# borodark/exmc

Hardware: AMD Instinct MI355X
Metric: leapfrog_steps_per_s (higher is better)
Workload: dtype f64; 1 GPU; eight_schools d=10, 4096 chains/GPU (4096 total), 138450 draws/chain (2769 steps of 50 draws) after one shared 1000-iteration warmup, max_tree_depth 10, target_accept 0.8; draws_per_chain=138450, lanes_per_chain=16, warmup_lanes_per_chain=16, seed=42

## Files before the change

### exmc_amd/csrc/exmc_device.hpp

```cpp
#pragma once

#include <hip/hip_runtime.h>
#include <stdint.h>
#include <type_traits>

#include <utility>

#include "../../include/exmc_detmath.h"

namespace exmc {

constexpr uint64_t kMask58 = (1ULL << 58) - 1;

#ifndef EXMC_FIXED_PART_PIECES
#define EXMC_FIXED_PART_PIECES 7
#endif

__device__ __forceinline__ bool div_in_range(double x) {
  const uint32_t h = (uint32_t)__double2hiint(x) & 0x7fffffffu;
  return (h - 0x28300000u) < (0x57C00000u - 0x28300000u);
}

struct Recip {
  double b, r;
};

__device__ __forceinline__ Recip make_recip(double b) { return Recip{b, exmc_rcp_refined(b)}; }

__device__ __forceinline__ Recip make_recip_literal(double b) {
  __asm__ volatile("" : "+v"(b));
  return make_recip(b);
}

template <bool kFast>
struct Div {
  bool ok = true;
  __device__ __forceinline__ void watch(double x) {
    if (kFast) ok = ok && div_in_range(x);
  }
  __device__ __forceinline__ void watch_if(bool relevant, double x) {
    if (kFast) ok = ok && (!relevant || div_in_range(x));
  }
  template <int ELO, int EHI>
  __device__ __forceinline__ void watch_exp_if(bool relevant, double x) {
    static_assert(ELO >= -380 && EHI <= 380 && ELO < EHI, "inside the division window");
    if (kFast) {
      const uint32_t h = (uint32_t)__double2hiint(x) & 0x7fffffffu;
      const bool in = (h - ((uint32_t)(1023 + ELO) << 20)) < ((uint32_t)(EHI - ELO) << 20);
      ok = ok && (!relevant || in);
    }
  }
  __device__ __forceinline__ double operator()(double a, const Recip& c) const {
    return kFast ? exmc_div_core(a, c.b, c.r) : (a / c.b);
  }
  __device__ __forceinline__ double operator()(double a, double b) const {
    return kFast ? exmc_div_core(a, b, exmc_rcp_refined(b)) : (a / b);
  }
};

template <class F>
__device__ __forceinline__ double with_fast_div(F&& f) {
  Div<true> fast;
  double r = f(fast);
  if (__builtin_expect(__any(fast.ok ? 0 : 1) != 0, 0)) {
    Div<false> exact;
    r = f(exact);
  }
  return r;
}

constexpr int kDppXor1 = 0xB1;
constexpr int kDppXor2 = 0x4E;
constexpr int kDppHalfMirror = 0x141;
constexpr int kDppRowMirror = 0x140;

template <int CTRL>
__device__ __forceinline__ double dpp_move(double v) {
  int lo = __double2loint(v), hi = __double2hiint(v);
  lo = __builtin_amdgcn_mov_dpp(lo, CTRL, 0xF, 0xF, true);
  hi = __builtin_amdgcn_mov_dpp(hi, CTRL, 0xF, 0xF, true);
  return __hiloint2double(hi, lo);
}

__device__ __forceinline__ double readlane_f64(double v, int lane) {
  int lo = __builtin_amdgcn_readlane(__double2loint(v), lane);
  int hi = __builtin_amdgcn_readlane(__double2hiint(v), lane);
  return __hiloint2double(hi, lo);
}

template <int G, int N>
__device__ __forceinline__ void xgroup_sum_n(double (&s)[N]) {
  static_assert(G == 16 || G == 32, "two or four lane groups per wavefront");
#pragma unroll
  for (int k = 0; k < N; k++) {
    double t = readlane_f64(s[k], 0);
#pragma unroll
    for (int j = 1; j < 64 / G; j++) t = t + readlane_f64(s[k], j * G);
    s[k] = t;
  }
}

#ifndef EXMC_XROW_PERMLANE
#define EXMC_XROW_PERMLANE 1
#endif
__device__ __forceinline__ double sum_xor16(double v) {
#if EXMC_XROW_PERMLANE
  const unsigned lo = (unsigned)__double2loint(v), hi = (unsigned)__double2hiint(v);
  const auto rl = __builtin_amdgcn_permlane16_swap(lo, lo, false, false);
  const auto rh = __builtin_amdgcn_permlane16_swap(hi, hi, false, false);
  return __hiloint2double((int)rh[0], (int)rl[0]) + __hiloint2double((int)rh[1], (int)rl[1]);
#else
  const int a = (((int)threadIdx.x & 63) ^ 16) << 2;
  return v + __hiloint2double(__builtin_amdgcn_ds_bpermute(a, __double2hiint(v)),
                              __builtin_amdgcn_ds_bpermute(a, __double2loint(v)));
#endif
}
__device__ __forceinline__ double sum_xor32(double v) {
#if EXMC_XROW_PERMLANE
  const unsigned lo = (unsigned)__double2loint(v), hi = (unsigned)__double2hiint(v);
  const auto rl = __builtin_amdgcn_permlane32_swap(lo, lo, false, false);
  const auto rh = __builtin_amdgcn_permlane32_swap(hi, hi, false, false);
  return __hiloint2double((int)rh[0], (int)rl[0]) + __hiloint2double((int)rh[1], (int)rl[1]);
#else
  const int a = (((int)threadIdx.x & 63) ^ 32) << 2;
  return v + __hiloint2double(__builtin_amdgcn_ds_bpermute(a, __double2hiint(v)),
                              __builtin_amdgcn_ds_bpermute(a, __double2loint(v)));
#endif
}
__device__ __forceinline__ double swap_xor16(double v) {
#if EXMC_XROW_PERMLANE
  const unsigned lo = (unsigned)__double2loint(v), hi = (unsigned)__double2hiint(v);
  const auto rl = __builtin_amdgcn_permlane16_swap(lo, lo, false, false);
  const auto rh = __builtin_amdgcn_permlane16_swap(hi, hi, false, false);
  return (threadIdx.x & 16) ? __hiloint2double((int)rh[0], (int)rl[0]) : __hiloint2double((int)rh[1], (int)rl[1]);
#else
  const int a = (((int)threadIdx.x & 63) ^ 16) << 2;
  return __hiloint2double(__builtin_amdgcn_ds_bpermute(a, __double2hiint(v)),
                          __builtin_amdgcn_ds_bpermute(a, __double2loint(v)));
#endif
}
__device__ __forceinline__ double swap_xor32(double v) {
#if EXMC_XROW_PERMLANE
  const unsigned lo = (unsigned)__double2loint(v), hi = (unsigned)__double2hiint(v);
  const auto rl = __builtin_amdgcn_permlane32_swap(lo, lo, false, false);
  const auto rh = __builtin_amdgcn_permlane32_swap(hi, hi, false, false);
  return (threadIdx.x & 32) ? __hiloint2double((int)rh[0], (int)rl[0]) : __hiloint2double((int)rh[1], (int)rl[1]);
#else
  const int a = (((int)threadIdx.x & 63) ^ 32) << 2;
  return __hiloint2double(__builtin_amdgcn_ds_bpermute(a, __double2hiint(v)),
                          __builtin_amdgcn_ds_bpermute(a, __double2loint(v)));
#endif
}

template <int N>
__device__ __forceinline__ void wave_scan_fwd(double (&v)[N]) {
  const int lane = threadIdx.x & 63, lr = lane & 15;
#define EXMC_SCAN_STAGE(DD)                                                       \
  _Pragma("unroll") for (int k = 0; k < N; k++) {                               \
    const double m = dpp_move<0x110 + DD>(v[k]);                  \
    v[k] = (lr >= DD) ? v[k] + m : v[k];                                          \
// ... 105 lines not shown
#endif
}

template <int G, bool kLds = false>
__device__ __forceinline__ double group_allsum(double v) {
  double a[1] = {v};
  group_allsum_n<G, 1, kLds>(a);
  return a[0];
}

template <int G, int D>
inline constexpr bool kSeqSum = (G == 16 && D <= 12);

#define EXMC_FMAC_B(A, V, I) \
  "v_fmac_f64_dpp %[" #A "], %[" #V "], %[one] row_newbcast:" #I " row_mask:0xf bank_mask:0xf\n\t"
#define EXMC_SEQ1(I) EXMC_FMAC_B(a0, v0, I)
#define EXMC_SEQ2(I) EXMC_SEQ1(I) EXMC_FMAC_B(a1, v1, I)
#define EXMC_SEQ3(I) EXMC_SEQ2(I) EXMC_FMAC_B(a2, v2, I)
#define EXMC_SEQ6(I) EXMC_SEQ3(I) EXMC_FMAC_B(a3, v3, I) EXMC_FMAC_B(a4, v4, I) EXMC_FMAC_B(a5, v5, I)
#define EXMC_LANES_1(S) S(0)
#define EXMC_LANES_2(S) EXMC_LANES_1(S) S(1)
#define EXMC_LANES_3(S) EXMC_LANES_2(S) S(2)
#define EXMC_LANES_4(S) EXMC_LANES_3(S) S(3)
#define EXMC_LANES_5(S) EXMC_LANES_4(S) S(4)
#define EXMC_LANES_6(S) EXMC_LANES_5(S) S(5)
#define EXMC_LANES_7(S) EXMC_LANES_6(S) S(6)
#define EXMC_LANES_8(S) EXMC_LANES_7(S) S(7)
#define EXMC_LANES_9(S) EXMC_LANES_8(S) S(8)
#define EXMC_LANES_10(S) EXMC_LANES_9(S) S(9)
#define EXMC_LANES_11(S) EXMC_LANES_10(S) S(10)
#define EXMC_LANES_12(S) EXMC_LANES_11(S) S(11)
#define EXMC_SEQSUM_ASM_H(HEAD, SEQ, OUTS, INS)                                              \
  if constexpr (NL == 1) __asm__(HEAD EXMC_LANES_1(SEQ) : OUTS : INS);                         \
  else if constexpr (NL == 2) __asm__(HEAD EXMC_LANES_2(SEQ) : OUTS : INS);                    \
  else if constexpr (NL == 3) __asm__(HEAD EXMC_LANES_3(SEQ) : OUTS : INS);                    \
  else if constexpr (NL == 4) __asm__(HEAD EXMC_LANES_4(SEQ) : OUTS : INS);                    \
  else if constexpr (NL == 5) __asm__(HEAD EXMC_LANES_5(SEQ) : OUTS : INS);                    \
  else if constexpr (NL == 6) __asm__(HEAD EXMC_LANES_6(SEQ) : OUTS : INS);                    \
  else if constexpr (NL == 7) __asm__(HEAD EXMC_LANES_7(SEQ) : OUTS : INS);                    \
  else if constexpr (NL == 8) __asm__(HEAD EXMC_LANES_8(SEQ) : OUTS : INS);                    \
  else if constexpr (NL == 9) __asm__(HEAD EXMC_LANES_9(SEQ) : OUTS : INS);                    \
  else if constexpr (NL == 10) __asm__(HEAD EXMC_LANES_10(SEQ) : OUTS : INS);                  \
  else if constexpr (NL == 11) __asm__(HEAD EXMC_LANES_11(SEQ) : OUTS : INS);                  \
  else __asm__(HEAD EXMC_LANES_12(SEQ) : OUTS : INS);
#define EXMC_NOP2 "s_nop 1\n\t"
#define EXMC_COMMA ,

__device__ __forceinline__ double seq_one() { return 1.0; }

template <int NL>
__device__ __forceinline__ void row_seqsum(double& a0, double v0) {
  static_assert(NL >= 1 && NL <= 12, "lanes of one DPP row, where the chain beats the butterfly");
  const double one = seq_one();
  EXMC_SEQSUM_ASM_H(EXMC_NOP2, EXMC_SEQ1, [a0] "+v"(a0), [v0] "v"(v0) EXMC_COMMA [one] "v"(one))
}
template <int NL>
__device__ __forceinline__ void row_seqsum(double& a0, double& a1, double v0, double v1) {
  const double one = seq_one();
  EXMC_SEQSUM_ASM_H(EXMC_NOP2, EXMC_SEQ2, [a0] "+v"(a0) EXMC_COMMA [a1] "+v"(a1),
                  [v0] "v"(v0) EXMC_COMMA [v1] "v"(v1) EXMC_COMMA [one] "v"(one))
}
template <int NL>
__device__ __forceinline__ void row_seqsum(double& a0, double& a1, double& a2, double v0, double v1,
                                           double v2) {
  const double one = seq_one();
  EXMC_SEQSUM_ASM_H(EXMC_NOP2, EXMC_SEQ3, [a0] "+v"(a0) EXMC_COMMA [a1] "+v"(a1) EXMC_COMMA [a2] "+v"(a2),
                  [v0] "v"(v0) EXMC_COMMA [v1] "v"(v1) EXMC_COMMA [v2] "v"(v2) EXMC_COMMA [one] "v"(one))
}
#define EXMC_FMAC_R(A, V, I) \
  "v_fmac_f64_dpp %[" #A "], %[" #V "], %[one] row_newbcast:%[l" #I "] row_mask:0xf bank_mask:0xf\n\t"
#define EXMC_SEQ3R(I) EXMC_FMAC_R(a0, v0, I) EXMC_FMAC_R(a1, v1, I) EXMC_FMAC_R(a2, v2, I)
#define EXMC_LANE_R(I) [l##I] "n"((I0 + I) & 15)
template <int I0, int NL>
__device__ __forceinline__ void row_seqsum_lanes(double& a0, double& a1, double& a2, double v0, double v1,
                                                 double v2) {
  static_assert(I0 >= 0 && NL >= 1 && NL <= 12 && I0 + NL <= 16, "a lane range of one DPP row");
  const double one = seq_one();
  EXMC_SEQSUM_ASM_H(EXMC_NOP2, EXMC_SEQ3R, [a0] "+v"(a0) EXMC_COMMA [a1] "+v"(a1) EXMC_COMMA [a2] "+v"(a2),
                  [v0] "v"(v0) EXMC_COMMA [v1] "v"(v1) EXMC_COMMA [v2] "v"(v2) EXMC_COMMA [one] "v"(one) EXMC_COMMA
                  EXMC_LANE_R(0) EXMC_COMMA EXMC_LANE_R(1) EXMC_COMMA EXMC_LANE_R(2) EXMC_COMMA EXMC_LANE_R(3) EXMC_COMMA
                  EXMC_LANE_R(4) EXMC_COMMA EXMC_LANE_R(5) EXMC_COMMA EXMC_LANE_R(6) EXMC_COMMA EXMC_LANE_R(7) EXMC_COMMA
                  EXMC_LANE_R(8) EXMC_COMMA EXMC_LANE_R(9) EXMC_COMMA EXMC_LANE_R(10) EXMC_COMMA EXMC_LANE_R(11))
}
#ifndef EXMC_ROW_SUM_PIECES
#define EXMC_ROW_SUM_PIECES 7
#endif
#define EXMC_ZERO_B(A) "v_mov_b64 %[" #A "], 0\n\t"
inline constexpr bool kZeroInBlock = (EXMC_FIXED_PART_PIECES & 4) != 0;
template <int NL>
__device__ __forceinline__ void row_seqsum_zero(double& a0, double& a1, double v0, double v1) {
  if constexpr (kZeroInBlock) {
    const double one = seq_one();
    EXMC_SEQSUM_ASM_H(EXMC_ZERO_B(a0) EXMC_ZERO_B(a1), EXMC_SEQ2, [a0] "=&v"(a0) EXMC_COMMA [a1] "=&v"(a1),
                      [v0] "v"(v0) EXMC_COMMA [v1] "v"(v1) EXMC_COMMA [one] "v"(one))
  } else {
    a0 = a1 = 0.0;
    row_seqsum<NL>(a0, a1, v0, v1);
  }
}
template <int I0, int NL>
__device__ __forceinline__ void row_seqsum_lanes_zero(double& a0, double& a1, double& a2, double v0, double v1,
                                                      double v2) {
  if constexpr (kZeroInBlock) {
    const double one = seq_one();
    EXMC_SEQSUM_ASM_H(EXMC_ZERO_B(a0) EXMC_ZERO_B(a1) EXMC_ZERO_B(a2), EXMC_SEQ3R,
                      [a0] "=&v"(a0) EXMC_COMMA [a1] "=&v"(a1) EXMC_COMMA [a2] "=&v"(a2),
                      [v0] "v"(v0) EXMC_COMMA [v1] "v"(v1) EXMC_COMMA [v2] "v"(v2) EXMC_COMMA [one] "v"(one) EXMC_COMMA
                      EXMC_LANE_R(0) EXMC_COMMA EXMC_LANE_R(1) EXMC_COMMA EXMC_LANE_R(2) EXMC_COMMA EXMC_LANE_R(3) EXMC_COMMA
                      EXMC_LANE_R(4) EXMC_COMMA EXMC_LANE_R(5) EXMC_COMMA EXMC_LANE_R(6) EXMC_COMMA EXMC_LANE_R(7) EXMC_COMMA
                      EXMC_LANE_R(8) EXMC_COMMA EXMC_LANE_R(9) EXMC_COMMA EXMC_LANE_R(10) EXMC_COMMA EXMC_LANE_R(11))
  } else {
    a0 = a1 = a2 = 0.0;
    row_seqsum_lanes<I0, NL>(a0, a1, a2, v0, v1, v2);
  }
}
#define EXMC_MV1(I) \
  "v_fmac_f64_dpp %[acc], %[x], %[c" #I "] row_newbcast:" #I " row_mask:0xf bank_mask:0xf\n\t"
template <int NL>
__device__ __forceinline__ double row_matvec(double x, const double (&c)[NL]) {
  static_assert(NL >= 1 && NL <= 12, "lanes of one DPP row");
  double acc = 0.0;
#define EXMC_MV_C(I) [c##I] "v"(c[(I) < NL ? (I) : 0])
  EXMC_SEQSUM_ASM_H(EXMC_NOP2, EXMC_MV1, [acc] "+v"(acc),
                  [x] "v"(x) EXMC_COMMA EXMC_MV_C(0) EXMC_COMMA EXMC_MV_C(1) EXMC_COMMA EXMC_MV_C(2) EXMC_COMMA
                  EXMC_MV_C(3) EXMC_COMMA EXMC_MV_C(4) EXMC_COMMA EXMC_MV_C(5) EXMC_COMMA EXMC_MV_C(6) EXMC_COMMA
                  EXMC_MV_C(7) EXMC_COMMA EXMC_MV_C(8) EXMC_COMMA EXMC_MV_C(9) EXMC_COMMA EXMC_MV_C(10) EXMC_COMMA
                  EXMC_MV_C(11))
#undef EXMC_MV_C
  return acc;
}
#define EXMC_OUTER1(I) \
  "v_fmac_f64_dpp %[m" #I "], %[x], %[c] row_newbcast:" #I " row_mask:0xf bank_mask:0xf\n\t"
template <int NL>
__device__ __forceinline__ void row_outer_acc(double (&m)[NL], double x, double c) {
  static_assert(NL >= 1 && NL <= 12, "lanes of one DPP row");
  double pad[12];
#pragma unroll
  for (int j = 0; j < 12; j++) pad[j] = (j < NL) ? m[j < NL ? j : 0] : 0.0;
#define EXMC_OUTER_M(I) [m##I] "+v"(pad[I])
  EXMC_SEQSUM_ASM_H(EXMC_NOP2, EXMC_OUTER1,
                  EXMC_OUTER_M(0) EXMC_COMMA EXMC_OUTER_M(1) EXMC_COMMA EXMC_OUTER_M(2) EXMC_COMMA EXMC_OUTER_M(3) EXMC_COMMA
                  EXMC_OUTER_M(4) EXMC_COMMA EXMC_OUTER_M(5) EXMC_COMMA EXMC_OUTER_M(6) EXMC_COMMA EXMC_OUTER_M(7) EXMC_COMMA
                  EXMC_OUTER_M(8) EXMC_COMMA EXMC_OUTER_M(9) EXMC_COMMA EXMC_OUTER_M(10) EXMC_COMMA EXMC_OUTER_M(11),
                  [x] "v"(x) EXMC_COMMA [c] "v"(c))
#undef EXMC_OUTER_M
#pragma unroll
  for (int j = 0; j < NL; j++) m[j] = pad[j];
}
template <int J>
__device__ __forceinline__ double row_bcast_f64(double x) {
  double acc = 0.0;
  const double one = seq_one();
  __asm__("s_nop 1\n\tv_fmac_f64_dpp %0, %1, %2 row_newbcast:%3 row_mask:0xf bank_mask:0xf"
          : "+v"(acc) : "v"(x), "v"(one), "n"(J));
  return acc;
}

template <int NL>
__device__ __forceinline__ void row_seqsum6(double (&a)[6], const double (&v)[6]) {
  const double one = seq_one();
  EXMC_SEQSUM_ASM_H(EXMC_NOP2, EXMC_SEQ6,
                  [a0] "+v"(a[0]) EXMC_COMMA [a1] "+v"(a[1]) EXMC_COMMA [a2] "+v"(a[2]) EXMC_COMMA
                  [a3] "+v"(a[3]) EXMC_COMMA [a4] "+v"(a[4]) EXMC_COMMA [a5] "+v"(a[5]),
                  [v0] "v"(v[0]) EXMC_COMMA [v1] "v"(v[1]) EXMC_COMMA [v2] "v"(v[2]) EXMC_COMMA
                  [v3] "v"(v[3]) EXMC_COMMA [v4] "v"(v[4]) EXMC_COMMA [v5] "v"(v[5]) EXMC_COMMA
                  [one] "v"(one))
// ... 724 lines not shown
```

### exmc_amd/csrc/exmc_models.hpp

```cpp
#pragma once

#include "exmc_device.hpp"

namespace exmc {

__device__ __forceinline__ double clamp200(double z) { return fmax(-200.0, fmin(z, 200.0)); }

struct ModelDefaults {
  static constexpr bool kVregMath = false;
  static constexpr bool kCoop = false;
  static constexpr int kExtraLdsDoubles = 0;
  static constexpr int kStageDoubles = 0;
  template <class C>
  __host__ static bool stage_ok(const C&) { return true; }
  static constexpr int kStageRowOffset = 0;
  static constexpr int kLdsDataDoubles = 0;
  static constexpr bool kPipeWarmup = true;
  static constexpr bool kHasPipeWarmup = true;
  static constexpr bool kXRowLds = false;
  static constexpr bool kRowDense = false;
  static constexpr bool kLaneDense = false;
  static constexpr bool kDenseImage = false;
  static constexpr int kDenseLdsDoubles = 0;
  static constexpr int kNutsWavesPerSimd = 1;
  static constexpr bool kRngOrbit = false;
  static constexpr bool kMigrate = false;
  static constexpr double kPrioRateWith = 1.0, kPrioRateWithout = 1.0;
  static constexpr int kPipeNutsLevels = 0;
  static constexpr bool kNutsZigInLds = true;
  static constexpr bool kRegradProposal = false;
  static constexpr int kWgWaves = 0;
  static constexpr int kWgLdsLevels = 1;
  static constexpr int kWgImageDoubles = 0;
  template <class C>
  __host__ __device__ static bool wg_ok(const C&) { return false; }
  static constexpr bool kLeafPairs = false;
  static constexpr bool kLeafPairExp = false;
  static constexpr bool kLeanMomentum = false;
  static constexpr bool kPassExpPairs = false;
  static constexpr bool kOuterLogPair = false;
  static constexpr bool kTreePrefix = false;
  static constexpr bool kRngWindow = false;
  static constexpr bool kPackedTrace = false;
};

extern __shared__ double exmc_dyn_lds[];
typedef double exmc_v2d __attribute__((ext_vector_type(2)));
typedef __attribute__((address_space(3))) exmc_v2d lds_v2d;
typedef __attribute__((address_space(3))) double lds_f64_m;
static __device__ const double exmc_logtab_dev[2 * EXMC_LOGTAB_ENTRIES] = {EXMC_LOGTAB_VALUES};
__device__ static __forceinline__ double exmc_log_tab_global(double x) {
  double m;
  int e;
  const int i = exmc_logtab_split(x, &m, &e);
  return exmc_logtab_finish(m, e, exmc_logtab_dev[2 * i], exmc_logtab_dev[2 * i + 1]);
}

struct EightSchoolsConsts {
  double y[8], sg[8], lsg[8];
  double c_mu;
  double c_hc;
  double c1;
};

template <int G>
struct EightSchools : ModelDefaults {
  static constexpr int D = 10;
  static constexpr int DPL = (D + G - 1) / G;
  static constexpr bool kVregMath = (DPL <= 2);
#ifndef EXMC_ES_PIPE_LEVELS
#define EXMC_ES_PIPE_LEVELS 2
#endif
  static constexpr int kPipeNutsLevels = (G == 16) ? EXMC_ES_PIPE_LEVELS : 0;
  static constexpr bool kLeafPairs = (G == 16);
  static constexpr bool kLeafPairExp = (G == 16);
  static constexpr bool kLeanMomentum = (G == 16);
  static constexpr bool kOuterLogPair = (G == 16);
  static constexpr bool kTreePrefix = (G == 16);
  static constexpr bool kRngWindow = (G == 16);
  static constexpr bool kPackedTrace = (G == 16);
  using MM = Math<kVregMath>;
  using Consts = EightSchoolsConsts;
  struct Lane {
    double y[DPL], lsg[DPL];
    Recip sg[DPL];
    Recip five;
    double cc;
  };

  __device__ static __forceinline__ void load(const Consts& c, int l, Lane& ln) {
#pragma unroll
    for (int k = 0; k < DPL; k++) {
      const int i = l + k * G;
      const int j = (i >= 2 && i < D) ? (i - 2) : 0;
      ln.y[k] = c.y[j];
      ln.sg[k] = make_recip(c.sg[j]);
      ln.lsg[k] = c.lsg[j];
    }
    ln.five = make_recip_literal(5.0);
    ln.cc = (l == 0) ? c.c_mu : c.c1;
  }

  __device__ static __forceinline__ double logp_grad(const Consts& c, const Lane& ln, int l,
                                                     const double (&q)[DPL], double (&g)[DPL]) {
    return with_fast_div([&](auto& dv) -> double { return eval(c, ln, l, q, g, dv); });
  }

  template <class DV>
  __device__ static __forceinline__ double eval(const Consts& c, const Lane& ln, int l,
                                                const double (&q)[DPL], double (&g)[DPL], DV& dv) {
    if constexpr (kSeqSum<G, D>) return eval_row(c, ln, l, q, g, dv);
    else return eval_slots(c, ln, l, q, g, dv);
  }

  struct Mid {
    double den, zc, T, lik;
  };
  template <class DV>
  __device__ static __forceinline__ void eval_row_grad(const Consts& c, const Lane& ln, int l,
                                                       const double (&q)[DPL], double (&g)[DPL], DV& dv,
                                                       Mid& m) {
    static_assert(DPL == 1, "one dimension per lane");
    const double mu = group_bcast_c<G, 0>(q[0]);
    const double zraw = group_bcast_c<G, 1>(q[0]);
    const double zc = clamp200(zraw);
    const double tau = MM::exp_pm200(zc);
    const bool isth = (l >= 2) && (l < D);
    const bool l0 = (l == 0), l1 = (l == 1);
    const double th = q[0];
    const double theta = mu + tau * th;
    const double resid = ln.y[0] - theta;
    constexpr bool kThetaLanes = (EXMC_ROW_SUM_PIECES & 1) != 0, kOneWatch = (EXMC_ROW_SUM_PIECES & 4) != 0;
    if constexpr (!kOneWatch) dv.watch_if(isth, resid);
    dv.watch_if(isth, ln.sg[0].b);
    const double z = dv(resid, ln.sg[0]);
    const double a = dv(z, ln.sg[0]);
    const double Lk = (-0.5 * (z * z)) - ln.lsg[0];
    const double Ak = a;
    const double Bk = a * th;
    double lik = 0.0, sa = 0.0, sb = 0.0;
    if constexpr (kThetaLanes) row_seqsum_lanes_zero<2, D - 2>(lik, sa, sb, Lk, Ak, Bk);
    else row_seqsum<D>(lik, sa, sb, isth ? Lk : 0.0, isth ? Ak : 0.0, isth ? Bk : 0.0);
    const double x = l0 ? (mu - 0.0) : tau;
    if constexpr (kOneWatch) dv.watch_if(isth || l0, l0 ? x : resid);
    else dv.watch_if(l0, x);
    const double zh = dv(x, ln.five);
    const double zh2 = zh * zh;
    const double w = dv(zh, ln.five);
    const double den = 1.0 + zh2;
    const double dhc = -dv(2.0 * w, den);
    const bool in = (zraw > -200.0) && (zraw < 200.0);
    double g_tau = in ? ((dhc + sb) * tau + 1.0) : 0.0;
    __asm__("" : "+v"(g_tau));
    const double g_mu = (-w) + sa;
    const double g_th = (-th) + a * tau;
    const double u2 = l0 ? zh2 : (th * th);
    g[0] = l0 ? g_mu : (l1 ? g_tau : g_th);
    m.den = den;
    m.zc = zc;
    m.T = -0.5 * (u2 + ln.cc);
    m.lik = lik;
  }
  __device__ static __forceinline__ double eval_row_finish(const Consts& c, int l, const Mid& m, double lg) {
    double t_tau = (c.c_hc - lg) + m.zc;
    __asm__("" : "+v"(t_tau));
    const double T = (l == 1) ? t_tau : m.T;
    const double Tv[1] = {T};
    const bool valid[1] = {l < D};
    return group_sum_slots<G, DPL, D>(Tv, valid, l, m.lik);
  }
  template <class DV>
  __device__ static __forceinline__ double eval_row(const Consts& c, const Lane& ln, int l,
                                                    const double (&q)[DPL], double (&g)[DPL], DV& dv) {
    Mid m;
    eval_row_grad(c, ln, l, q, g, dv, m);
    return eval_row_finish(c, l, m, MM::log_ge1(m.den));
  }

  template <class DV>
  __device__ static __forceinline__ double eval_slots(const Consts& c, const Lane& ln, int l,
                                                      const double (&q)[DPL], double (&g)[DPL], DV& dv) {
    const double mu = group_bcast_c<G, 0 % G>(q[0 / G]);
    const double zraw = group_bcast_c<G, 1 % G>(q[1 / G]);
    const double zc = clamp200(zraw);
    const double tau = MM::exp_pm200(zc);
    dv.watch(mu);
    double L[DPL], A[DPL], B[DPL], T[DPL];
    bool valid[DPL];
#pragma unroll
    for (int k = 0; k < DPL; k++) {
      const int i = l + k * G;
      valid[k] = i < D;
      const bool isth = (i >= 2) && (i < D);
      const double th = q[k];
      const double theta = mu + tau * th;
      const double resid = ln.y[k] - theta;
      dv.watch_if(isth, resid);
      dv.watch_if(isth, ln.sg[k].b);
      const double z = dv(resid, ln.sg[k]);
      const double a = dv(z, ln.sg[k]);
      L[k] = isth ? ((-0.5 * (z * z)) - ln.lsg[k]) : 0.0;
      A[k] = isth ? a : 0.0;
      B[k] = isth ? (a * th) : 0.0;
      T[k] = -0.5 * (th * th + c.c1);
      g[k] = (-th) + a * tau;
    }
    double s3[3] = {0.0, 0.0, 0.0};
    if constexpr (kSeqSum<G, D>) {
      row_seqsum<D>(s3[0], s3[1], s3[2], L[0], A[0], B[0]);
    } else {
#pragma unroll
      for (int k = 0; k < DPL; k++) {
        s3[0] = valid[k] ? (s3[0] + L[k]) : s3[0];
        s3[1] = valid[k] ? (s3[1] + A[k]) : s3[1];
        s3[2] = valid[k] ? (s3[2] + B[k]) : s3[2];
      }
      group_allsum_n<G, 3>(s3);
    }
    const double lik = s3[0], sa = s3[1], sb = s3[2];
    const double zmu = dv(mu - 0.0, ln.five);
    const double t_mu = -0.5 * (zmu * zmu + c.c_mu);
    const double zt = dv(tau, ln.five);
    const double zt2 = zt * zt;
    const double t_tau = (c.c_hc - MM::log_ge1(1.0 + zt2)) + zc;
    const double g_mu = (-dv(zmu, ln.five)) + sa;
    const double dhc = -dv(dv(2.0 * zt, ln.five), 1.0 + zt2);
    const bool in = (zraw > -200.0) && (zraw < 200.0);
    const double g_tau = in ? ((dhc + sb) * tau + 1.0) : 0.0;
#pragma unroll
    for (int k = 0; k < DPL; k++) {
      const int i = l + k * G;
      if (i == 0) { T[k] = t_mu; g[k] = g_mu; }
      if (i == 1) { T[k] = t_tau; g[k] = g_tau; }
    }
    return group_sum_slots<G, DPL, D>(T, valid, l, lik);
  }
};

struct SimpleConsts {
  double y[64];
  int n;
  double c_mu;
  double log2pi32;
  double tiny32;
};

template <int G>
struct Simple : ModelDefaults {
  static_assert(G == 1, "simple model is one lane per chain");
  static constexpr int D = 2;
  static constexpr int DPL = 2;
  using Consts = SimpleConsts;
  struct Lane {};
  __device__ static __forceinline__ void load(const Consts&, int, Lane&) {}
  __device__ static __forceinline__ double logp_grad(const Consts& c, const Lane&, int,
                                                     const double (&q)[DPL], double (&g)[DPL]) {
    const double mu = q[0], zc = clamp200(q[1]);
    const double sigma = exmc_exp(zc);
    const double ss = fmax(sigma, c.tiny32);
    const double ls = exmc_log(ss);
    const double zmu = (mu - 0.0) / 5.0;
// ... 1014 lines not shown
          __builtin_amdgcn_sched_barrier(0);
          exmc_wait_lgkm0();
#pragma unroll
          for (int j = 0; j < kAhead - 1; j++) sj = sj + v[j];
        }
        sj_own[k] = sj;
      }
    } else {
#pragma unroll
      for (int k = 0; k < DPL; k++) {
        double lik = 0.0, f = 0.0, z2s = 0.0, sj = 0.0;
        for (int i = ln.i0[k]; i < ln.i1[k]; i++) sj = sj + obs(alpha_own[k], c.fl[i], c.y[i], lik, f, z2s);
        sj_own[k] = sj;
        if (valid[k]) {
          s[0] = s[0] + lik;
          s[4] = s[4] + f;
          s[5] = s[5] + z2s;
        }
      }
    }
#pragma unroll
    for (int k = 0; k < DPL; k++) {
      const double ar = q[k];
      const double sj = sj_own[k];
      if (valid[k]) {
        s[1] = s[1] + sj;
        s[2] = s[2] + sj * ln.u[k];
        s[3] = s[3] + sj * ar;
      }
      T[k] = -0.5 * (ar * ar + ln.kc[kC1]);
      g[k] = (-ar) + sj * sa;
    }
    if constexpr (G == 64) rs64_allsum6(s);
    else group_allsum_n<G, 6>(s);
    const bool in_a = (zsa_raw > -200.0) && (zsa_raw < 200.0);
    const bool in_y = (zsy_raw > -200.0) && (zsy_raw < 200.0);
    if constexpr (kSpread) {
      constexpr int ks = J / G;
      const int j = l + ks * G;
      const bool is_mu = j == J, is_g = j == J + 1, is_a = j == J + 2, is_y = j == J + 3, is_b = j == J + 4;
      const double v = is_mu ? mu : (is_g ? gam : beta);
      Recip rc;
      rc.b = is_mu ? ln.ten.b : ln.five.b;
      rc.r = is_mu ? ln.ten.r : ln.five.r;
      const double cst = is_mu ? ln.kc[kMu10] : ln.kc[kN5];
      const double sx = is_mu ? s[1] : (is_g ? s[2] : s[4]);
      const double zn = dv(v - 0.0, rc);
      const double Tn = -0.5 * (zn * zn + cst);
      const double gn = (-dv(zn, rc)) + sx;
      const double zc = is_a ? za : zy, zc2 = is_a ? za2 : zy2;
      const double dc = -dv(dv(2.0 * zc, ln.c25), 1.0 + zc2);
      const double ga = in_a ? ((dc + s[3]) * sa + 1.0) : 0.0;
      const double gy = in_y ? ((dc * sy + s[5]) + 1.0) : 0.0;
      const bool is_n = is_mu || is_g || is_b;
      T[ks] = is_n ? Tn : (is_a ? t_sa : (is_y ? t_sy : T[ks]));
      g[ks] = is_n ? gn : (is_a ? ga : (is_y ? gy : g[ks]));
#pragma unroll
      for (int k = 0; k < DPL; k++)
        if (l + k * G >= D) g[k] = 0.0;
      return group_sum_slots<G, DPL>(T, valid, l, s[0]);
    }
    const double zmu = dv(mu - 0.0, ln.ten), zg = dv(gam - 0.0, ln.five), zb = dv(beta - 0.0, ln.five);
#pragma unroll
    for (int k = 0; k < DPL; k++) {
      const int j = l + k * G;
      if (j == J) { T[k] = -0.5 * (zmu * zmu + ln.kc[kMu10]); g[k] = (-dv(zmu, ln.ten)) + s[1]; }
      if (j == J + 1) { T[k] = -0.5 * (zg * zg + ln.kc[kN5]); g[k] = (-dv(zg, ln.five)) + s[2]; }
      if (j == J + 2) { T[k] = t_sa; g[k] = in_a ? ((dsa + s[3]) * sa + 1.0) : 0.0; }
      if (j == J + 3) { T[k] = t_sy; g[k] = in_y ? ((dsy * sy + s[5]) + 1.0) : 0.0; }
      if (j == J + 4) { T[k] = -0.5 * (zb * zb + ln.kc[kN5]); g[k] = (-dv(zb, ln.five)) + s[4]; }
      if (j >= D) g[k] = 0.0;
    }
    return group_sum_slots<G, DPL>(T, valid, l, s[0]);
  }
};

template <class M>
struct RowDenseModel : M {
  static constexpr bool kRowDense = true;
  static constexpr bool kPipeWarmup = false;
  static constexpr bool kOuterLogPair = false;
  static constexpr bool kTreePrefix = false;
  static constexpr bool kRngWindow = false;
  static constexpr bool kPackedTrace = false;
  static_assert(M::DPL == 1 && M::D <= 12, "row layout: one dimension per lane, D <= 12");
};

template <class M, int G>
struct LaneDenseModel : M {
  static constexpr bool kLaneDense = true;
  static constexpr bool kPipeWarmup = false;
  static constexpr int kNutsWavesPerSimd = 1;
  static constexpr int kPipeNutsLevels = 0;
  static constexpr bool kDenseImage = M::D * M::D * 8 <= 16 * 1024;
  static constexpr int kDenseLdsDoubles = (64 / G) * 3 * M::D + (kDenseImage ? M::D * M::D + 64 : 0);
  static_assert(G >= 16 && M::DPL * G >= M::D && !M::kCoop, "a lane layout that holds the whole chain");
};

}

#ifdef EXMC_CUSTOM_HEADER
#define EXMC_GEN_HOST static inline
#define EXMC_GEN_FN static __host__ __device__ __forceinline__
static __host__ __device__ __noinline__ double exmc_gen_exp_call(double x) { return exmc_exp(x); }
static __host__ __device__ __noinline__ double exmc_gen_log_call(double x) { return exmc_log(x); }
static __host__ __device__ __noinline__ double exmc_gen_log1p_call(double x) { return exmc_log1p(x); }
static __host__ __device__ __noinline__ double exmc_gen_erf_call(double x) { return exmc_erf(x); }
#define EXMC_GEN_ERF exmc_gen_erf_call
#define EXMC_GENV_ERF exmc_gen_erf_call
#ifdef EXMC_GEN_INLINE_MATH
#define EXMC_GEN_EXP exmc_exp
#define EXMC_GEN_LOG exmc_log
#define EXMC_GEN_LOG1P exmc_log1p
#else
#define EXMC_GEN_EXP exmc_gen_exp_call
#define EXMC_GEN_LOG exmc_gen_log_call
#define EXMC_GEN_LOG1P exmc_gen_log1p_call
#endif
#ifdef EXMC_GENV_CALLED_MATH
#define EXMC_GENV_EXP exmc_gen_exp_call
#define EXMC_GENV_LOG exmc_gen_log_call
#define EXMC_GENV_LOG1P exmc_gen_log1p_call
#else
#define EXMC_GENV_EXP exmc_exp
#define EXMC_GENV_LOG exmc_log
#define EXMC_GENV_LOG1P exmc_log1p
#endif
#ifdef EXMC_GENL_CALLED_MATH
#define EXMC_GENL_EXP exmc_gen_exp_call
#define EXMC_GENL_LOG exmc_gen_log_call
#define EXMC_GENL_LOG1P exmc_gen_log1p_call
#else
#define EXMC_GENL_EXP exmc::Math<true>::exp
#define EXMC_GENL_LOG exmc::Math<true>::log
#define EXMC_GENL_LOG1P exmc_log1p
#endif
#define EXMC_GENL_ERF exmc_gen_erf_call
#define EXMC_GEN_CTX_DECL , int shoff
#define EXMC_GEN_SH(i) exmc::exmc_dyn_lds[shoff + (i)]
#define EXMC_GEN_XROW (EXMC_GEN_LANES == 64 && EXMC_GEN_WAVES_PER_SIMD == 2)
#define EXMC_GEN_ALLSUM(s) exmc::group_allsum_n<EXMC_GEN_LANES, EXMC_GEN_NS, EXMC_GEN_XROW>(s)
#define EXMC_GEN_ALLSUM_W(w) exmc::group_allsum_n<EXMC_GEN_LANES, EXMC_GEN_NW, EXMC_GEN_XROW>(w)
#define EXMC_GEN_BATCH_LOG(n, b) exmc::lane_batch<EXMC_GEN_LANES, n>(b, l, [](double a_) { return EXMC_GENL_LOG(a_); })
#define EXMC_GEN_BATCH_EXP(n, b) exmc::lane_batch<EXMC_GEN_LANES, n>(b, l, [](double a_) { return EXMC_GENL_EXP(a_); })
#define EXMC_GEN_BATCH_LOG1P(n, b) exmc::lane_batch<EXMC_GEN_LANES, n>(b, l, [](double a_) { return EXMC_GENL_LOG1P(a_); })
#define EXMC_GEN_BATCH_RCP(n, b) exmc::lane_batch<EXMC_GEN_LANES, n>(b, l, [](double a_) { return 1.0 / a_; })
#define EXMC_GEN_FENCE() exmc::wave_lds_fence()
#define EXMC_GEN_SCAN_FWD(N, v, m, zo, h, sg, wo)                              \
  do {                                                                        \
    exmc::wave_scan_fwd<N>(v);                                                \
    _Pragma("unroll") for (int k_ = 0; k_ < (N); k_++)                        \
      if (l + 64 * k_ <= (m)) EXMC_GEN_SH((wo) + l + 64 * k_) = (v)[k_];     \
    exmc::wave_lds_fence();                                                   \
  } while (0)
#define EXMC_GEN_SCAN_BWD(N, v, m, zo, sg, we, ww, ga, sz, a0)                 \
  do {                                                                        \
    exmc::wave_scan_bwd<N>(v);                                                \
    double p_[1] = {0.0};                                                     \
    _Pragma("unroll") for (int k_ = 0; k_ < (N); k_++) {                      \
      const int e_ = l + 64 * k_;                                             \
      const bool in_ = e_ >= 1 && e_ <= (m);                                  \
      const double z_ = EXMC_GEN_SH(EXMC_GEN_IT((zo) + e_));                  \
      if (in_) EXMC_GEN_SH((ga) + e_) = (sg) * (v)[k_];                       \
      p_[0] = in_ ? p_[0] + z_ * (v)[k_] : p_[0];                             \
    }                                                                         \
    exmc::group_allsum_n<64, 1, EXMC_GEN_XROW>(p_);                           \
// ... 379 lines not shown
```

### exmc_amd/csrc/exmc_nuts.hpp

```cpp
#pragma once

#include <type_traits>

#include "exmc_models.hpp"

#ifndef EXMC_ABLATE
#define EXMC_ABLATE 0
#endif

#ifndef EXMC_PROFILE_SECTIONS
#define EXMC_PROFILE_SECTIONS 0
#endif

namespace exmc {

#ifdef EXMC_XCC_PROBE
__device__ double g_wave_probe[4096 * 5];
#endif

#if EXMC_PROFILE_SECTIONS
__device__ unsigned long long g_prof[16];
#define EXMC_PROF_DECL long long prof_[10] = {0, 0, 0, 0, 0, 0, 0, 0, 0, 0}; long long prof_t_ = clock64();
#define EXMC_PROF(i) { const long long n_ = clock64(); prof_[i] += n_ - prof_t_; prof_t_ = n_; }
#define EXMC_PROF_COUNT(i) { prof_[i] += 1; }
// ... 1113 lines not shown
    bool stopped = false;
    for (int i = 1; i < nunit; i++) {
      unit(eps_dir, true);
      EXMC_IPROF(1)
      pb.sync();
      EXMC_IPROF(2)
      if (__any(pb.get_alive() ? 1 : 0) == 0) { stopped = true; break; }
    }
    if (stopped) continue;
#pragma unroll
    for (int k = 0; k < DPL; k++) {
      if (go_right) { qR[k] = q[k]; pR[k] = p[k]; gR[k] = g[k]; }
      else { qL[k] = q[k]; pL[k] = p[k]; gL[k] = g[k]; }
    }
    const int nleaf = 1 << depth;
    for (int i = 0; i < nleaf; i++) rng_advance(prng);
    go_right = rng_uniform(prng) > 0.5;
#pragma unroll
    for (int k = 0; k < DPL; k++) {
      q[k] = go_right ? qR[k] : qL[k];
      p[k] = go_right ? pR[k] : pL[k];
      g[k] = go_right ? gR[k] : gL[k];
    }
    EXMC_IPROF(3)
    unit(go_right ? eps : -eps, true);
    EXMC_IPROF(1)
  }
  {
    double z[DPL];
    const Rng before = next_rng;
    draw_momentum_variates<M, G>(L, next_rng, z);
    pb.put_momentum(z, before, next_rng);
  }
  EXMC_IPROF(3)
  pb.sync();
  EXMC_IPROF(2)
  EXMC_IPROF_FLUSH
  return true;
}

template <int DPL>
struct TreeTop {
  double (&qL)[DPL], (&pL)[DPL], (&gL)[DPL], (&qR)[DPL], (&pR)[DPL], (&gR)[DPL];
  double (&rho)[DPL], (&qp)[DPL], (&gp)[DPL];
  double &logpP, &lsw, &acc;
  int &n, &depth;
  bool &div, &turn, &alive;
};

struct NoRngWindow {
  static constexpr int kOff = 0;
};
template <int I>
using IntC = std::integral_constant<int, I>;

template <class M, int G, class Win = NoRngWindow>
__device__ __forceinline__ void tree_prefix(const typename M::Consts& mc, const NutsLane<M, G>& L,
                                            double eps, double jlp0, int max_depth, Rng& trng,
                                            TreeTop<M::DPL> T, double (&q)[M::DPL], double (&p)[M::DPL],
                                            double (&g)[M::DPL], Win* win = nullptr) {
  constexpr int DPL = M::DPL;
  using MM = Math<M::kVregMath>;
  static_assert(G >= 11, "one lane per argument of the widest batch");
  static_assert(!M::kRegradProposal, "the proposal's gradient travels with it");
  constexpr bool kWin = !std::is_same<Win, NoRngWindow>::value;
  double u[10];
  double ul = 0.0;
  if constexpr (kWin) {
    static_assert(G == 16, "a group is one DPP row");
    win->build(trng);
    ul = (double)(rng_scramble(win->own()) >> 5) * 0x1p-53;
    trng = win->template state<10>();
  } else {
#pragma unroll
    for (int i = 0; i < 10; i++) u[i] = rng_uniform(trng);
  }
  auto U = [&](auto ic) -> double {
    constexpr int I = decltype(ic)::value;
    if constexpr (kWin) return group_bcast_c<G, Win::kOff + I>(ul);
    else return u[I];
  };
  const bool r0 = U(IntC<0>{}) > 0.5, r1 = U(IntC<2>{}) > 0.5, r2 = U(IntC<5>{}) > 0.5;

  PipeLeaf<DPL> f0, f1, f2, f3, f4, f5, f6;
  auto leap = [&](double eps_dir, PipeLeaf<DPL>& lf) {
    const double h = eps_dir / 2.0;
#pragma unroll
    for (int k = 0; k < DPL; k++) p[k] = p[k] + h * g[k];
    mass_drift<M, G>(L, eps_dir, p, q);
    lf.logp = M::logp_grad(mc, L.ln, L.l, q, g);
#pragma unroll
    for (int k = 0; k < DPL; k++) p[k] = p[k] + h * g[k];
#pragma unroll
    for (int k = 0; k < DPL; k++) { lf.q[k] = q[k]; lf.p[k] = p[k]; lf.g[k] = g[k]; }
  };
  double q1[DPL], g1[DPL], q2[DPL], g2[DPL];
#pragma unroll
  for (int k = 0; k < DPL; k++) { q[k] = T.qL[k]; p[k] = T.pL[k]; g[k] = T.gL[k]; }
  leap(r0 ? eps : -eps, f0);
  const bool same01 = (r0 == r1), same12 = (r1 == r2);
#pragma unroll
  for (int k = 0; k < DPL; k++) {
    q[k] = q1[k] = same01 ? f0.q[k] : T.qL[k];
    p[k] = same01 ? f0.p[k] : T.pL[k];
    g[k] = g1[k] = same01 ? f0.g[k] : T.gL[k];
  }
  leap(r1 ? eps : -eps, f1);
  leap(r1 ? eps : -eps, f2);
#pragma unroll
  for (int k = 0; k < DPL; k++) {
    q[k] = q2[k] = same12 ? f2.q[k] : (same01 ? T.qL[k] : f0.q[k]);
    p[k] = same12 ? f2.p[k] : (same01 ? T.pL[k] : f0.p[k]);
    g[k] = g2[k] = same12 ? f2.g[k] : (same01 ? T.gL[k] : f0.g[k]);
  }
  leap(r2 ? eps : -eps, f3);
  leap(r2 ? eps : -eps, f4);
  leap(r2 ? eps : -eps, f5);
  leap(r2 ? eps : -eps, f6);

  auto scalars = [&](PipeLeaf<DPL>& lf) -> double {
    const double jlp = lf.logp - mass_ke<M, G>(L, lf.p);
    const bool fin = exmc_isfinite(jlp);
    const double dl = jlp - jlp0;
    lf.div = fin ? (dl < -1000.0) : true;
    lf.lsw = fin ? dl : -1001.0;
    return fmin(dl, 0.0);
  };
  double x[11];
  x[0] = scalars(f0); x[1] = scalars(f1); x[2] = scalars(f2); x[3] = scalars(f3);
  x[4] = scalars(f4); x[5] = scalars(f5); x[6] = scalars(f6);
  x[7] = MM::lse_arg(f1.lsw, f2.lsw);
  x[8] = MM::lse_arg(f3.lsw, f4.lsw);
  x[9] = MM::lse_arg(f5.lsw, f6.lsw);
  x[10] = MM::lse_arg(T.lsw, f0.lsw);
  lane_batch<G>(x, L.l, [](double v) { return MM::exp_le0(v); });
  auto accept = [&](PipeLeaf<DPL>& lf, double ex) { lf.acc = lf.div ? 0.0 : fmin(1.0, ex); };
  accept(f0, x[0]); accept(f1, x[1]); accept(f2, x[2]); accept(f3, x[3]);
  accept(f4, x[4]); accept(f5, x[5]); accept(f6, x[6]);

  double y[11] = {1.0 + x[7], 1.0 + x[8], 1.0 + x[9], 1.0 + x[10], 0.0, 0.0, 0.0, 0.0, 0.0, 0.0, 0.0};
  if constexpr (kWin) {
    constexpr int o = Win::kOff;
    const int l = L.l;
    const bool ge1 = (l == o) || (l == o + 2) || (l == o + 5) || (l == o + 10);
    double a = ul;
    a = (l == o) ? y[0] : a;
    a = (l == o + 2) ? y[1] : a;
    a = (l == o + 5) ? y[2] : a;
    a = (l == o + 10) ? y[3] : a;
    const double r = MM::log_main(a);
    const double v = ge1 ? exmc_log_ge1_fix(a, r) : exmc_log_unit_fix(a, r);
    y[0] = group_bcast_c<G, o>(v);
    y[1] = group_bcast_c<G, o + 2>(v);
    y[2] = group_bcast_c<G, o + 5>(v);
    y[3] = group_bcast_c<G, o + 10>(v);
    y[4] = group_bcast_c<G, o + 1>(v);
    y[5] = group_bcast_c<G, o + 3>(v);
    y[6] = group_bcast_c<G, o + 4>(v);
    y[7] = group_bcast_c<G, o + 6>(v);
    y[8] = group_bcast_c<G, o + 7>(v);
    y[9] = group_bcast_c<G, o + 8>(v);
    y[10] = group_bcast_c<G, o + 9>(v);
  } else {
    y[4] = u[1]; y[5] = u[3]; y[6] = u[4]; y[7] = u[6]; y[8] = u[7]; y[9] = u[8]; y[10] = u[9];
    double v[11];
#pragma unroll
    for (int i = 0; i < 11; i++) v[i] = y[i];
    lane_batch<G>(y, L.l, [](double a) { return MM::log_main(a); });
#pragma unroll
    for (int i = 0; i < 4; i++) y[i] = exmc_log_ge1_fix(v[i], y[i]);
#pragma unroll
    for (int i = 4; i < 11; i++) y[i] = exmc_log_unit_fix(v[i], y[i]);
  }
  const double lsw12 = MM::lse_finish(f1.lsw, f2.lsw, y[0]);
  const double lsw34 = MM::lse_finish(f3.lsw, f4.lsw, y[1]);
  const double lsw56 = MM::lse_finish(f5.lsw, f6.lsw, y[2]);
  const double c12 = f1.div ? f1.lsw : lsw12;
  const double c34 = f3.div ? f3.lsw : lsw34;
  const double c56 = f5.div ? f5.lsw : lsw56;

  auto outer = [&](const PipeUnit<DPL>& c, bool go_right, double log1pe, double logu, auto dc) {
    constexpr int depth = decltype(dc)::value;
    constexpr bool kOneTest = depth == 0 && (EXMC_ROW_SUM_PIECES & 2) != 0;
    if (!T.alive) return;
    const double lsw = MM::lse_finish(T.lsw, c.lsw, log1pe);
    const bool use_sub = logu < (c.lsw - T.lsw);
    if (use_sub) {
      T.logpP = c.logpP;
#pragma unroll
      for (int k = 0; k < DPL; k++) { T.qp[k] = c.qp[k]; T.gp[k] = c.gp[k]; }
    }
    const bool divg = T.div || c.div;
    bool turning = divg || c.turn;
    double rho[DPL];
#pragma unroll
    for (int k = 0; k < DPL; k++) rho[k] = T.rho[k] + c.rho[k];
    if (!turning) {
      double nearp[DPL], farp[DPL];
#pragma unroll
      for (int k = 0; k < DPL; k++) {
        nearp[k] = go_right ? T.pR[k] : T.pL[k];
// ... 1722 lines not shown
```

Baseline: 3.850 billion leapfrog_steps/s.

## Batch the per-leaf log across idle lanes and defer the logp reduction

```diff
diff --git a/exmc_amd/csrc/exmc_device.hpp b/exmc_amd/csrc/exmc_device.hpp
--- a/exmc_amd/csrc/exmc_device.hpp
+++ b/exmc_amd/csrc/exmc_device.hpp
@@ -74,8 +74,17 @@
 constexpr int kDppHalfMirror = 0x141;
 constexpr int kDppRowMirror = 0x140;
 
+#ifndef EXMC_PREFIX_FINISH_PIECES
+#define EXMC_PREFIX_FINISH_PIECES 3
+#endif
+
 template <int CTRL>
 __device__ __forceinline__ double dpp_move(double v) {
+  if constexpr (CTRL >= 0x150 && CTRL <= 0x15F && (EXMC_PREFIX_FINISH_PIECES & 1) != 0) {
+    long long b = __double_as_longlong(v);
+    b = __builtin_amdgcn_update_dpp(b, b, CTRL, 0xF, 0xF, true);
+    return __longlong_as_double(b);
+  }
   int lo = __double2loint(v), hi = __double2hiint(v);
   lo = __builtin_amdgcn_mov_dpp(lo, CTRL, 0xF, 0xF, true);
   hi = __builtin_amdgcn_mov_dpp(hi, CTRL, 0xF, 0xF, true);
@@ -347,6 +356,17 @@
                   EXMC_LANE_R(4) EXMC_COMMA EXMC_LANE_R(5) EXMC_COMMA EXMC_LANE_R(6) EXMC_COMMA EXMC_LANE_R(7) EXMC_COMMA
                   EXMC_LANE_R(8) EXMC_COMMA EXMC_LANE_R(9) EXMC_COMMA EXMC_LANE_R(10) EXMC_COMMA EXMC_LANE_R(11))
 }
+#define EXMC_SEQ1R(I) EXMC_FMAC_R(a0, v0, I)
+template <int I0, int NL>
+__device__ __forceinline__ void row_seqsum_lanes(double& a0, double v0) {
+  static_assert(I0 >= 0 && NL >= 1 && NL <= 12 && I0 + NL <= 16, "a lane range of one DPP row");
+  const double one = seq_one();
+  EXMC_SEQSUM_ASM_H(EXMC_NOP2, EXMC_SEQ1R, [a0] "+v"(a0),
+                  [v0] "v"(v0) EXMC_COMMA [one] "v"(one) EXMC_COMMA
+                  EXMC_LANE_R(0) EXMC_COMMA EXMC_LANE_R(1) EXMC_COMMA EXMC_LANE_R(2) EXMC_COMMA EXMC_LANE_R(3) EXMC_COMMA
+                  EXMC_LANE_R(4) EXMC_COMMA EXMC_LANE_R(5) EXMC_COMMA EXMC_LANE_R(6) EXMC_COMMA EXMC_LANE_R(7) EXMC_COMMA
+                  EXMC_LANE_R(8) EXMC_COMMA EXMC_LANE_R(9) EXMC_COMMA EXMC_LANE_R(10) EXMC_COMMA EXMC_LANE_R(11))
+}
 #ifndef EXMC_ROW_SUM_PIECES
 #define EXMC_ROW_SUM_PIECES 7
 #endif
diff --git a/exmc_amd/csrc/exmc_models.hpp b/exmc_amd/csrc/exmc_models.hpp
--- a/exmc_amd/csrc/exmc_models.hpp
+++ b/exmc_amd/csrc/exmc_models.hpp
@@ -42,6 +42,7 @@
   static constexpr bool kTreePrefix = false;
   static constexpr bool kRngWindow = false;
   static constexpr bool kPackedTrace = false;
+  static constexpr bool kPrefixLogBatch = false;
 };
 
 extern __shared__ double exmc_dyn_lds[];
@@ -177,6 +178,29 @@
     return eval_row_finish(c, l, m, MM::log_ge1(m.den));
   }
 
+  static constexpr bool kPrefixLogBatch = (G == 16);
+  static constexpr int kPreLogLanes = (G == 16) ? 1 + (G - D) : 0;
+  __device__ static constexpr int pre_log_lane(int k) { return k == 0 ? 1 : D + k - 1; }
+  __device__ static __forceinline__ double logp_grad_pre(const Consts& c, const Lane& ln, int l,
+                                                         const double (&q)[DPL], double (&g)[DPL]) {
+    static_assert(kSeqSum<G, D>, "the row form");
+    return with_fast_div([&](auto& dv) -> double {
+      Mid m;
+      eval_row_grad(c, ln, l, q, g, dv, m);
+      const double head = m.lik + m.T;
+      return (l == 0) ? head : (((l >= 2) && (l < D)) ? m.T : m.den);
+    });
+  }
+  __device__ static __forceinline__ double logp_finish(const Consts& c, int l, const double (&q)[DPL],
+                                                       double pre, double lg) {
+    double t_tau = (c.c_hc - lg) + clamp200(q[0]);
+    __asm__("" : "+v"(t_tau));
+    const double T = (l == 1) ? t_tau : pre;
+    double acc = group_bcast_c<G, 0>(pre);
+    row_seqsum_lanes<1, D - 1>(acc, T);
+    return acc;
+  }
+
   template <class DV>
   __device__ static __forceinline__ double eval_slots(const Consts& c, const Lane& ln, int l,
                                                       const double (&q)[DPL], double (&g)[DPL], DV& dv) {
@@ -1357,6 +1381,7 @@
   static constexpr bool kOuterLogPair = false;
   static constexpr bool kTreePrefix = false;
   static constexpr bool kRngWindow = false;
+  static constexpr bool kPrefixLogBatch = false;
   static constexpr bool kPackedTrace = false;
   static_assert(M::DPL == 1 && M::D <= 12, "row layout: one dimension per lane, D <= 12");
 };
diff --git a/exmc_amd/csrc/exmc_nuts.hpp b/exmc_amd/csrc/exmc_nuts.hpp
--- a/exmc_amd/csrc/exmc_nuts.hpp
+++ b/exmc_amd/csrc/exmc_nuts.hpp
@@ -1219,13 +1219,21 @@
   };
   const bool r0 = U(IntC<0>{}) > 0.5, r1 = U(IntC<2>{}) > 0.5, r2 = U(IntC<5>{}) > 0.5;
 
+  constexpr bool kSplitLogp = M::kPrefixLogBatch && (EXMC_PREFIX_FINISH_PIECES & 6) != 0;
+  constexpr bool kLogBatch = kSplitLogp && (EXMC_PREFIX_FINISH_PIECES & 2) != 0;
   PipeLeaf<DPL> f0, f1, f2, f3, f4, f5, f6;
   auto leap = [&](double eps_dir, PipeLeaf<DPL>& lf) {
     const double h = eps_dir / 2.0;
 #pragma unroll
     for (int k = 0; k < DPL; k++) p[k] = p[k] + h * g[k];
     mass_drift<M, G>(L, eps_dir, p, q);
-    lf.logp = M::logp_grad(mc, L.ln, L.l, q, g);
+    if constexpr (kSplitLogp) {
+      lf.logp = M::logp_grad_pre(mc, L.ln, L.l, q, g);
+      if constexpr (!kLogBatch)
+        lf.logp = M::logp_finish(mc, L.l, q, lf.logp, MM::log_ge1(group_bcast_c<G, M::pre_log_lane(0)>(lf.logp)));
+    } else {
+      lf.logp = M::logp_grad(mc, L.ln, L.l, q, g);
+    }
 #pragma unroll
     for (int k = 0; k < DPL; k++) p[k] = p[k] + h * g[k];
 #pragma unroll
@@ -1254,6 +1262,24 @@
   leap(r2 ? eps : -eps, f4);
   leap(r2 ? eps : -eps, f5);
   leap(r2 ? eps : -eps, f6);
+
+  if constexpr (kLogBatch) {
+    static_assert(M::kPreLogLanes >= 7, "a lane per leaf of the unit");
+    const int l = L.l;
+    double a = f0.logp;
+    a = (l == M::pre_log_lane(1)) ? f1.logp : a;
+    a = (l == M::pre_log_lane(2)) ? f2.logp : a;
+    a = (l == M::pre_log_lane(3)) ? f3.logp : a;
+    a = (l == M::pre_log_lane(4)) ? f4.logp : a;
+    a = (l == M::pre_log_lane(5)) ? f5.logp : a;
+    a = (l == M::pre_log_lane(6)) ? f6.logp : a;
+    const double v = MM::log_ge1(a);
+    auto finish = [&](PipeLeaf<DPL>& lf, auto ic) {
+      lf.logp = M::logp_finish(mc, l, lf.q, lf.logp, group_bcast_c<G, M::pre_log_lane(decltype(ic)::value)>(v));
+    };
+    finish(f0, IntC<0>{}); finish(f1, IntC<1>{}); finish(f2, IntC<2>{}); finish(f3, IntC<3>{});
+    finish(f4, IntC<4>{}); finish(f5, IntC<5>{}); finish(f6, IntC<6>{});
+  }
 
   auto scalars = [&](PipeLeaf<DPL>& lf) -> double {
     const double jlp = lf.logp - mass_ke<M, G>(L, lf.p);
```

Result: faster. 3.947 billion leapfrog_steps/s, median of 6 (+2.5%).
